# ChenyuWang-Monica/REED

Hardware: AMD Instinct MI355X
Metric: SiT-XL/2 ImageNet-256 train images/sec (higher is better)
Workload: dtype bf16

## Files before the change

include/reed_hip.h:

```cpp
#ifndef REED_HIP_H
#define REED_HIP_H
#include <stdint.h>
#ifdef __cplusplus
extern "C" {
#endif

const char* reed_last_error(void);
int reed_version(void);
int reed_half_kind(void);

int reed_gemm(int layout, int epilogue, const void* P, int64_t ldp, const void* Q, int64_t ldq,
              int M, int N, int K, void* C, int64_t ldc, void* C2, int64_t ldc2, const void* R,
              int64_t ldr, const void* bias, const void* gate, int64_t ldgate, int rows_per_gate,
              float* dbias, int accumulate, int split_k, int64_t slab_stride, void* stream);

int reed_wgrad_group(int n, const void* const* dy, const void* const* x, float* const* dw, float* const* dbias,
                     const int* n_out, const int* k_in, int tokens, int accumulate, void* stream);
int reed_wgrad_group_deal(int n, const int* n_out, const int* k_in, const int* has_bias, int cus, unsigned* items);

int reed_set_cu_reserve(int n);
int reed_planning_cus(void);
int reed_set_concurrent_comm(int on);

int reed_gemm_force_tile(int tile);
// ... 22 lines not shown

int reed_gate_bwd(const float* dx, const void* y, const void* gate, int64_t ldgate, void* dy,
                  float* part, float* part_dy, int M, int D, int T, void* stream);
int reed_transpose_bf16(const void* src, void* dst, int R, int C, void* stream);
int reed_rowsum_f32(const float* part, int R, float* ws, float* out, int N, int accumulate, void* stream);

int reed_reduce_mod_parts(const float* const* parts, const int64_t* strides, const int64_t* offs,
                          int nparts, void* dmod, int64_t lddmod, int B, int D, int chunks,
                          void* stream);

int reed_attention_fwd(const void* qkv, void* o, float* lse, int B, int T, int H, int hd,
                       void* stream);
int reed_attention_bwd(const void* qkv, const void* o, const void* d_o, const float* lse,
                       void* dqkv, int B, int T, int H, int hd, void* stream);
int64_t reed_attention_bwd_ws_floats(int B, int T, int H);
int reed_attention_bwd_ws(const void* qkv, const void* o, const void* d_o, const float* lse, void* dqkv, float* ws,
                          int B, int T, int H, int hd, void* stream);
int reed_attention_bwd_dp(const void* qkv, const void* d_o, const float* lse, const float* dpart, void* dqkv, float* ws,
                          int B, int T, int H, int hd, void* stream);

int reed_qk_norm_fwd(const void* qkv, const float* qw, const float* qb, const float* kw, const float* kb,
                     void* out, float* stats, int M, int H, int hd, float eps, void* stream);
int64_t reed_qk_norm_bwd_part_floats(int M, int H, int hd);
int reed_qk_norm_bwd(const void* dn, const void* qkv, const float* stats, const float* qw, const float* kw,
                     void* dpre, float* part, int M, int H, int hd, void* stream);

int reed_patch_embed_fwd(const float* x, const void* w, const void* bias, const float* pos,
                         float* tokens, int B, int C, int HW, int P, int D, void* stream);
int reed_patchify_bf16(const float* x, void* out, int B, int C, int HW, int P, int order, void* stream);
int64_t reed_smallk_wgrad_ws_floats(int Dw, int KS);
int reed_smallk_wgrad(const void* wide, int wide_is_f32, const void* small, float* ws, float* out,
                      float* colsum_wide, float* colsum_small, int M, int Dw, int KS, int layout,
                      int accumulate, void* stream);
int reed_timestep_sinusoid(const float* t, void* out, int B, int dim, float max_period, void* stream);
int reed_label_cond(const int64_t* labels, const uint8_t* drop, int num_classes, int table_rows, const float* table,
                    const void* t_emb, int64_t* labels_out, float* c, void* silu_c, int* err_flag, int B, int D,
                    void* stream);
int reed_label_cond_bwd(const float* dsilu_c, const float* c, const int64_t* labels_eff, void* dt_emb,
                        float* dtable, int B, int D, void* stream);
int reed_final_layer_fwd(const float* x, const void* shift, const void* scale, int64_t ldmod,
                         const void* w, const void* bias, float* out, float* mean, float* rstd,
                         int B, int T, int D, int C, int P, float eps, void* stream);
int reed_final_layer_bwd_rows(const float* dout, const float* x, const float* mean, const float* rstd,
                              const void* shift, const void* scale, int64_t ldmod, const void* w,
                              void* hbuf, void* dlin, void* dh, int B, int T, int D, int C, int P,
                              void* stream);
int reed_token_mean_fwd(const float* x, void* out, int B, int T, int D, void* stream);
int reed_token_mean_bwd(const void* dmean, float* dx, int B, int T, int D, void* stream);

int reed_sample_posterior(const float* moments, const float* eps, float* out, int B, int64_t half,
                          float scale, float bias, void* stream);
int reed_interpolant(const float* x, const float* noise, const float* t, float* xt, float* target,
                     int B, int64_t per, int path_type, void* stream);
int reed_mse_fwd(const float* out, const float* target, float* loss, int B, int64_t per, void* stream);
int reed_mse_bwd(const float* out, const float* target, const float* gscale, float* dout, int B,
                 int64_t per, void* stream);
int reed_cosine_fwd(const void* zt, const float* z, float* rowdot, float* loss, int B, int T, int Z,
                    void* stream);
int reed_cosine_bwd(const void* zt, const float* z, const float* gscale, void* dzt, int B, int T,
                    int Z, void* stream);

int reed_grad_sqnorm(const float* g, int64_t n, float* partial, int nblocks, void* stream);
int reed_clip_finalize(const float* partial, int nblocks, float max_norm, float* norm_clip, void* stream);
int reed_clip_finalize_scaled(const float* partial, int nblocks, float max_norm, float* norm_clip, float* scaler_state,
                              float growth_factor, float backoff_factor, float growth_interval, void* stream);
int reed_adamw_ema(float* p, const float* g, float* m, float* v, float* ema, void* shadow,
                   int64_t n_train, int64_t n_total, const float* norm_clip, const float* scaler_state, float lr,
                   float beta1, float beta2, float eps, float weight_decay, float bc1, float bc2, float ema_decay,
                   void* stream);
int reed_cast_bf16(const float* src, void* dst, int64_t n, void* stream);

int reed_sampler_update(const double* x_cur, const float* model_out, const double* d_prev,
                        double* d_store, double* x_next, int64_t n_elems, int cfg, double cfg_scale,
                        double dt, double w0, double w1, void* stream);
int reed_sde_update(const double* x_cur, const float* model_out, const double* eps, double* x_next,
// ... 51 lines not shown
```

reed_amd/csrc/embed.hip:

```cpp
#include "../../include/reed_hip.h"
#include "common.hpp"

namespace {

constexpr int MAXV = 5;
constexpr int NSL = 256;

__device__ __forceinline__ f32x4 ld_bf4(const bf16* p) {
  bf16x4 v = *(const bf16x4*)p;
  return f32x4{bf2f(v[0]), bf2f(v[1]), bf2f(v[2]), bf2f(v[3])};
}

__device__ __forceinline__ long patch_src(int b, int t, int k, int C, int HW, int P, int order) {
  const int G = HW / P, ph = t / G, pw = t - ph * G;
  int c, pi, pj;
  if (order == 0) { c = k / (P * P); int r = k - c * P * P; pi = r / P; pj = r - pi * P; }
  else { c = k % C; int r = k / C; pi = r / P; pj = r - pi * P; }
  return (((long)b * C + c) * HW + ph * P + pi) * HW + pw * P + pj;
}
__global__ __launch_bounds__(256) void patchify_kernel(const float* __restrict__ x, bf16* __restrict__ out, int B,
                                                       int C, int HW, int P, int order) {
  const int G = HW / P, T = G * G, K = C * P * P;
  long i = (long)blockIdx.x * 256 + threadIdx.x;
  if (i >= (long)B * T * K) return;
  int k = (int)(i % K);
  long bt = i / K;
  out[i] = f2bf(x[patch_src((int)(bt / T), (int)(bt % T), k, C, HW, P, order)]);
}

__global__ __launch_bounds__(256) void patch_embed_fwd_kernel(const float* __restrict__ x, const bf16* __restrict__ w,
                                                              const bf16* __restrict__ bias,
                                                              const float* __restrict__ pos, float* __restrict__ tok,
                                                              int B, int C, int HW, int P, int D) {
  extern __shared__ float xs[];
// ... 116 lines not shown
#pragma unroll
    for (int r = 0; r < RG; ++r) {
      ws0 += w0[r]; ws1 += w1[r];
#pragma unroll
      for (int c = 0; c < KSP / 8; ++c)
#pragma unroll
        for (int j = 0; j < 8; ++j) {
          const float f = bf2f(sv[r][c][j]);
          acc0[8 * c + j] = fmaf(w0[r], f, acc0[8 * c + j]);
          acc1[8 * c + j] = fmaf(w1[r], f, acc1[8 * c + j]);
        }
    }
  }
  if (dok) {
#pragma unroll
    for (int k = 0; k < KSP; ++k)
      if (k0 + k < KS) {
        const int kk = k0 + k;
        if (layout == 0) { wout[(long)d * KS + kk] = acc0[k]; wout[(long)(d + 1) * KS + kk] = acc1[k]; }
        else { wout[(long)kk * Dw + d] = acc0[k]; wout[(long)kk * Dw + d + 1] = acc1[k]; }
      }
    if (blockIdx.z == 0) {
      wout[(long)KS * Dw + d] = ws0;
      wout[(long)KS * Dw + d + 1] = ws1;
    }
  }
  if (blockIdx.x == 0 && blockIdx.z == 0) {
    for (int k = lane; k < KS; k += 64) {
      float ssum = 0.f;
      for (int m = mbeg; m < mend; ++m) ssum += bf2f(small[(long)m * KS + k]);
      wout[(long)KS * Dw + Dw + k] = ssum;
    }
  }
}
__global__ __launch_bounds__(256) void smallk_reduce_kernel(const float* __restrict__ ws, long stride,
                                                            float* __restrict__ o0, long n0, float* __restrict__ o1,
                                                            long n1, float* __restrict__ o2, long n2, int accumulate) {
  long i = (long)blockIdx.x * 256 + threadIdx.x;
  if (i >= n0 + n1 + n2) return;
  float* dst;
  if (i < n0) dst = o0 ? o0 + i : nullptr;
  else if (i < n0 + n1) dst = o1 ? o1 + (i - n0) : nullptr;
  else dst = o2 ? o2 + (i - n0 - n1) : nullptr;
  if (!dst) return;
  float s = accumulate ? *dst : 0.f;
  for (int z = 0; z < NSL; ++z) s += ws[(long)z * stride + i];
  *dst = s;
}

__global__ void sinusoid_kernel(const float* __restrict__ t, bf16* __restrict__ out, int B, int dim, float max_period) {
  const int half = dim / 2;
  int i = blockIdx.x * 256 + threadIdx.x;
  if (i >= B * half) return;
  int b = i / half, k = i - b * half;
  float a = (float)(-log((double)max_period)) * (float)k;
  float f = expf(a / (float)half);
  float arg = t[b] * f;
  out[(long)b * dim + k] = f2bf(cosf(arg));
  out[(long)b * dim + half + k] = f2bf(sinf(arg));
  if ((dim & 1) && k == 0) out[(long)b * dim + dim - 1] = f2bf(0.f);
}

__global__ void label_cond_kernel(const int64_t* __restrict__ labels, const uint8_t* __restrict__ drop, int num_classes,
                                  int table_rows, const float* __restrict__ table, const bf16* __restrict__ t_emb,
                                  int64_t* __restrict__ labels_out, float* __restrict__ c, bf16* __restrict__ silu_c,
                                  int* __restrict__ err, int D) {
  const int b = blockIdx.y, d = blockIdx.x * 256 + threadIdx.x;
  int64_t lab = labels[b];
  if (drop && drop[b]) lab = num_classes;
  if (lab < 0 || lab >= table_rows) {
    if (d == 0 && err) *err = 1;
    lab = 0;
  }
  if (d == 0 && labels_out) labels_out[b] = lab;
  if (d >= D) return;
  float v = bf2f(t_emb[(long)b * D + d]) + table[lab * D + d];
  c[(long)b * D + d] = v;
  silu_c[(long)b * D + d] = f2bf(silu_f(v));
}
__global__ void label_cond_bwd_kernel(const float* __restrict__ dsilu, const float* __restrict__ c,
                                      const int64_t* __restrict__ labels_eff, bf16* __restrict__ dt_emb,
                                      float* __restrict__ dtable, int B, int D) {
  const int d = blockIdx.x * 256 + threadIdx.x;
  if (d >= D) return;
  for (int b = 0; b < B; ++b) {
    float g = bfround(dsilu[(long)b * D + d]) * silu_grad_f(c[(long)b * D + d]);
    dt_emb[(long)b * D + d] = f2bf(g);
    dtable[labels_eff[b] * D + d] += g;
  }
}

__global__ __launch_bounds__(256) void final_fwd_kernel(const float* __restrict__ x, const bf16* __restrict__ shift,
                                                        const bf16* __restrict__ scale, long ldmod,
                                                        const bf16* __restrict__ w, const bf16* __restrict__ bias,
                                                        float* __restrict__ out, float* __restrict__ mean,
                                                        float* __restrict__ rstd, int B, int T, int D, int C, int P,
                                                        float eps) {
  const int row = blockIdx.x * 4 + (threadIdx.x >> 6);
  const int M = B * T;
  if (row >= M) return;
  const int lane = threadIdx.x & 63, nv = D >> 2;
  const float* xr = x + (long)row * D;
  f32x4 v[MAXV];
  float s = 0.f;
#pragma unroll
  for (int k = 0; k < MAXV; ++k) {
    int idx = lane + 64 * k;
    if (idx < nv) { v[k] = *(const f32x4*)(xr + idx * 4); s += v[k][0] + v[k][1] + v[k][2] + v[k][3]; }
  }
  const float mu = wave_sum(s) / D;
  float q = 0.f;
#pragma unroll
  for (int k = 0; k < MAXV; ++k) {
    int idx = lane + 64 * k;
    if (idx < nv) {
#pragma unroll
      for (int j = 0; j < 4; ++j) { float d = v[k][j] - mu; q += d * d; }
    }
  }
  const float r = rsqrtf(wave_sum(q) / D + eps);
  if (lane == 0 && mean) { mean[row] = mu; rstd[row] = r; }
// ... 77 lines not shown
      if (lane == 0 && mean && (u == 0 || two)) { mean[row] = mu[u]; rstd[row] = r[u]; }
      bb_[u] = row / T;
      tt_[u] = row - bb_[u] * T;
      const bf16* sc = scale + (long)bb_[u] * ldmod;
      const bf16* sh = shift + (long)bb_[u] * ldmod;
#pragma unroll
      for (int k = 0; k < MAXV; ++k) {
        int idx = lane + 64 * k;
        if (idx < nv) {
          f32x4 a = ld_bf4(sc + idx * 4), bb = ld_bf4(sh + idx * 4);
#pragma unroll
          for (int j = 0; j < 4; ++j) v[u][k][j] = bfround((v[u][k][j] - mu[u]) * r[u] * bfround(1.f + a[j]) + bb[j]);
        }
      }
    }
    for (int j = 0; j < NO; ++j) {
      float acc[2] = {0.f, 0.f};
#pragma unroll
      for (int k = 0; k < MAXV; ++k) {
        int idx = lane + 64 * k;
        if (idx < nv) {
          f32x4 wv = ld_bf4(wl + j * D + idx * 4);
#pragma unroll
          for (int u = 0; u < 2; ++u) acc[u] += v[u][k][0] * wv[0] + v[u][k][1] * wv[1] + v[u][k][2] * wv[2] + v[u][k][3] * wv[3];
        }
      }
#pragma unroll
      for (int u = 0; u < 2; ++u) acc[u] = wave_sum(acc[u]);
      if (lane == 0) {
        const float bj = bias ? bf2f(bias[j]) : 0.f;
        out[patch_src(bb_[0], tt_[0], j, C, HW, P, 1)] = bfround(acc[0] + bj);
        if (two) out[patch_src(bb_[1], tt_[1], j, C, HW, P, 1)] = bfround(acc[1] + bj);
      }
    }
  }
}

__global__ __launch_bounds__(256) void final_bwd_rows_kernel(const float* __restrict__ dout, const float* __restrict__ x,
                                                             const float* __restrict__ mean,
                                                             const float* __restrict__ rstd,
                                                             const bf16* __restrict__ shift,
                                                             const bf16* __restrict__ scale, long ldmod,
                                                             const bf16* __restrict__ w, bf16* __restrict__ hbuf,
                                                             bf16* __restrict__ dlin, bf16* __restrict__ dh, int B,
                                                             int T, int D, int C, int P) {
  extern __shared__ float dl[];
  const int wave = threadIdx.x >> 6, lane = threadIdx.x & 63, nv = D >> 2;
  const int row = blockIdx.x * 4 + wave;
  const int M = B * T, NO = P * P * C, HW = (int)(sqrtf((float)T) + 0.5f) * P;
  const bool ok = row < M;
  const int b = ok ? row / T : 0, t = ok ? row - b * T : 0;
  float* my = dl + wave * NO;
  if (ok) {
    for (int j = lane; j < NO; j += 64) {
      float g = bfround(dout[patch_src(b, t, j, C, HW, P, 1)]);
      my[j] = g;
      dlin[(long)row * NO + j] = f2bf(g);
    }
  }
  __syncthreads();
  if (!ok) return;
  const float mu = mean[row], r = rstd[row];
  const bf16* sc = scale + (long)b * ldmod;
  const bf16* sh = shift + (long)b * ldmod;
#pragma unroll
  for (int k = 0; k < MAXV; ++k) {
// ... 43 lines not shown
    }
    __builtin_amdgcn_wave_barrier();
    const float mu = mean[row], r = rstd[row];
    const bf16* sc = scale + (long)b * ldmod;
    const bf16* sh = shift + (long)b * ldmod;
#pragma unroll
    for (int k = 0; k < MAXV; ++k) {
      int idx = lane + 64 * k;
      if (idx < nv) {
        f32x4 xv = *(const f32x4*)(x + (long)row * D + idx * 4);
        f32x4 a = ld_bf4(sc + idx * 4), bb = ld_bf4(sh + idx * 4);
        bf16x4 hv, gv;
        f32x4 acc = {0, 0, 0, 0};
        for (int j = 0; j < NO; ++j) {
          f32x4 wv = ld_bf4(wl + j * D + idx * 4);
          float g = my[j];
          acc[0] += g * wv[0]; acc[1] += g * wv[1]; acc[2] += g * wv[2]; acc[3] += g * wv[3];
        }
#pragma unroll
        for (int j = 0; j < 4; ++j) {
          hv[j] = f2bf((xv[j] - mu) * r * bfround(1.f + a[j]) + bb[j]);
          gv[j] = f2bf(acc[j]);
        }
        *(bf16x4*)(hbuf + (long)row * D + idx * 4) = hv;
        *(bf16x4*)(dh + (long)row * D + idx * 4) = gv;
      }
    }
    __builtin_amdgcn_wave_barrier();
  }
}

}

extern "C" int reed_patchify_bf16(const float* x, void* out, int B, int C, int HW, int P, int order, void* stream) {
  REED_CHECK_ARG(HW % P == 0, "patchify: HW=%d not divisible by P=%d", HW, P);
  long n = (long)B * C * HW * HW;
  REED_KLAUNCH(patchify_kernel, dim3(cdiv(n, 256)), dim3(256), 0, (hipStream_t)stream, x, (bf16*)out, B, C, HW, P, order);
  REED_LAUNCH_CHECK();
  return REED_OK;
}

extern "C" int reed_patch_embed_fwd(const float* x, const void* w, const void* bias, const float* pos,
                                    float* tokens, int B, int C, int HW, int P, int D, void* stream) {
  REED_CHECK_ARG(x && w && pos && tokens, "patch_embed_fwd: null pointer");
  REED_CHECK_ARG(HW % P == 0 && (C * P * P) % 8 == 0, "patch_embed: HW=%d P=%d C=%d unsupported", HW, P, C);
  const int T = (HW / P) * (HW / P), K = C * P * P;
  if (K == PK && D % 4 == 0 && D <= 4 * PNT && ((uintptr_t)w % 16) == 0 && ((uintptr_t)pos % 16) == 0 &&
      ((uintptr_t)tokens % 16) == 0) {
    REED_KLAUNCH(patch_embed_fwd16_kernel, dim3(cdiv((long)B * T, PT)), dim3(PNT), 0, (hipStream_t)stream, x, (const bf16*)w,
                 (const bf16*)bias, pos, tokens, B, C, HW, P, D);
    REED_LAUNCH_CHECK();
    return REED_OK;
  }
  REED_KLAUNCH(patch_embed_fwd_kernel, dim3(cdiv((long)B * T, 8)), dim3(256), 8 * K * sizeof(float),
                     (hipStream_t)stream, x, (const bf16*)w, (const bf16*)bias, pos, tokens, B, C, HW, P, D);
  REED_LAUNCH_CHECK();
  return REED_OK;
}

extern "C" int64_t reed_smallk_wgrad_ws_floats(int Dw, int KS) { return (int64_t)NSL * ((int64_t)KS * Dw + Dw + KS); }

extern "C" int reed_smallk_wgrad(const void* wide, int wide_is_f32, const void* small, float* ws, float* out,
                                 float* colsum_wide, float* colsum_small, int M, int Dw, int KS, int layout,
                                 int accumulate, void* stream) {
  REED_CHECK_ARG(wide && small && ws, "smallk_wgrad: null pointer");
  REED_CHECK_ARG(KS >= 8 && KS <= 512 && KS % 8 == 0, "smallk_wgrad: KS=%d must be a multiple of 8 in 8..512", KS);
  REED_CHECK_ARG(Dw > 0 && Dw % 2 == 0, "smallk_wgrad: Dw=%d must be even", Dw);
  if (KS <= 16) {
    dim3 grid(cdiv(Dw, 128), NSL, 1);
    if (wide_is_f32) REED_KLAUNCH((smallk_wgrad_kernel<true, 16>), grid, dim3(64), 0, (hipStream_t)stream, wide, (const bf16*)small, ws, M, Dw, KS, layout);
    else REED_KLAUNCH((smallk_wgrad_kernel<false, 16>), grid, dim3(64), 0, (hipStream_t)stream, wide, (const bf16*)small, ws, M, Dw, KS, layout);
  } else {
    dim3 grid(cdiv(Dw, 128), NSL, cdiv(KS, 32));
    if (wide_is_f32) REED_KLAUNCH((smallk_wgrad_kernel<true, 32>), grid, dim3(64), 0, (hipStream_t)stream, wide, (const bf16*)small, ws, M, Dw, KS, layout);
    else REED_KLAUNCH((smallk_wgrad_kernel<false, 32>), grid, dim3(64), 0, (hipStream_t)stream, wide, (const bf16*)small, ws, M, Dw, KS, layout);
  }
  REED_LAUNCH_CHECK();
  long n0 = (long)KS * Dw, n1 = Dw, n2 = KS;
  REED_KLAUNCH(smallk_reduce_kernel, dim3(cdiv(n0 + n1 + n2, 256)), dim3(256), 0, (hipStream_t)stream, ws,
                     n0 + n1 + n2, out, n0, colsum_wide, n1, colsum_small, n2, accumulate);
  REED_LAUNCH_CHECK();
  return REED_OK;
}

extern "C" int reed_timestep_sinusoid(const float* t, void* out, int B, int dim, float max_period, void* stream) {
  REED_CHECK_ARG(t && out && dim >= 2, "timestep_sinusoid: bad args");
  REED_KLAUNCH(sinusoid_kernel, dim3(cdiv((long)B * (dim / 2), 256)), dim3(256), 0, (hipStream_t)stream, t,
                     (bf16*)out, B, dim, max_period);
  REED_LAUNCH_CHECK();
  return REED_OK;
}

extern "C" int reed_label_cond(const int64_t* labels, const uint8_t* drop, int num_classes, int table_rows,
                               const float* table, const void* t_emb, int64_t* labels_out, float* c, void* silu_c,
                               int* err_flag, int B, int D, void* stream) {
  REED_CHECK_ARG(labels && table && t_emb && c && silu_c, "label_cond: null pointer");
  REED_CHECK_ARG(table_rows >= 1 && (!drop || num_classes < table_rows),
                 "label_cond: label dropout needs a null-class row (num_classes < table_rows)");
  REED_KLAUNCH(label_cond_kernel, dim3(cdiv(D, 256), B), dim3(256), 0, (hipStream_t)stream, labels, drop,
                     num_classes, table_rows, table, (const bf16*)t_emb, labels_out, c, (bf16*)silu_c, err_flag, D);
  REED_LAUNCH_CHECK();
  return REED_OK;
}

extern "C" int reed_label_cond_bwd(const float* dsilu_c, const float* c, const int64_t* labels_eff, void* dt_emb,
                                   float* dtable, int B, int D, void* stream) {
  REED_CHECK_ARG(dsilu_c && c && labels_eff && dt_emb && dtable, "label_cond_bwd: null pointer");
  REED_KLAUNCH(label_cond_bwd_kernel, dim3(cdiv(D, 256)), dim3(256), 0, (hipStream_t)stream, dsilu_c, c,
                     labels_eff, (bf16*)dt_emb, dtable, B, D);
  REED_LAUNCH_CHECK();
  return REED_OK;
}

extern "C" int reed_final_layer_fwd(const float* x, const void* shift, const void* scale, int64_t ldmod,
                                    const void* w, const void* bias, float* out, float* mean, float* rstd,
                                    int B, int T, int D, int C, int P, float eps, void* stream) {
  REED_CHECK_ARG(x && shift && scale && w && out, "final_layer_fwd: null pointer");
  REED_CHECK_ARG(D % 4 == 0 && D <= 256 * MAXV, "final_layer: D=%d unsupported", D);
  int G = (int)(sqrtf((float)T) + 0.5f);
  REED_CHECK_ARG(G * G == T, "final_layer: T=%d is not a square grid", T);
  const long wbytes = (long)P * P * C * D * sizeof(bf16);
  if (wbytes <= 64 * 1024 && (P * P * C * D) % 8 == 0 && ((uintptr_t)w % 16) == 0) {
    REED_KLAUNCH(final_fwd_lds_kernel, dim3(cdiv((long)B * T, FR)), dim3(256), (size_t)wbytes, (hipStream_t)stream, x,
                 (const bf16*)shift, (const bf16*)scale, (long)ldmod, (const bf16*)w, (const bf16*)bias, out, mean, rstd, B, T, D, C, P,
                 eps);
    REED_LAUNCH_CHECK();
    return REED_OK;
  }
  REED_KLAUNCH(final_fwd_kernel, dim3(cdiv((long)B * T, 4)), dim3(256), 0, (hipStream_t)stream, x,
                     (const bf16*)shift, (const bf16*)scale, (long)ldmod, (const bf16*)w, (const bf16*)bias, out, mean,
                     rstd, B, T, D, C, P, eps);
  REED_LAUNCH_CHECK();
  return REED_OK;
}

extern "C" int reed_final_layer_bwd_rows(const float* dout, const float* x, const float* mean, const float* rstd,
                                         const void* shift, const void* scale, int64_t ldmod, const void* w,
                                         void* hbuf, void* dlin, void* dh, int B, int T, int D, int C, int P,
                                         void* stream) {
  REED_CHECK_ARG(dout && x && mean && rstd && shift && scale && w && hbuf && dlin && dh, "final_layer_bwd_rows: null pointer");
  REED_CHECK_ARG(D % 4 == 0 && D <= 256 * MAXV, "final_layer: D=%d unsupported", D);
  REED_CHECK_ARG(B > 0 && T > 0, "final_layer_bwd_rows: bad B=%d T=%d", B, T);
  int G = (int)(sqrtf((float)T) + 0.5f);
  REED_CHECK_ARG(G * G == T, "final_layer_bwd_rows: T=%d is not a square grid", T);
  const int NO = P * P * C;
  const long wb = (long)NO * D * sizeof(bf16);
  if (wb + 4 * NO * (long)sizeof(float) <= 64 * 1024 && (NO * D) % 8 == 0 && ((uintptr_t)w % 16) == 0) {
    REED_KLAUNCH(final_bwd_rows_lds_kernel, dim3(cdiv((long)B * T, FR)), dim3(256), (size_t)(wb + 4 * NO * sizeof(float)),
                 (hipStream_t)stream, dout, x, mean, rstd, (const bf16*)shift, (const bf16*)scale, (long)ldmod, (const bf16*)w,
                 (bf16*)hbuf, (bf16*)dlin, (bf16*)dh, B, T, D, C, P);
    REED_LAUNCH_CHECK();
    return REED_OK;
  }
  REED_KLAUNCH(final_bwd_rows_kernel, dim3(cdiv((long)B * T, 4)), dim3(256), 4 * NO * sizeof(float),
                     (hipStream_t)stream, dout, x, mean, rstd, (const bf16*)shift, (const bf16*)scale, (long)ldmod,
                     (const bf16*)w, (bf16*)hbuf, (bf16*)dlin, (bf16*)dh, B, T, D, C, P);
  REED_LAUNCH_CHECK();
  return REED_OK;
}
```

reed_amd/ops.py:

```python
import contextlib
import ctypes

import math

import torch

from . import _lib

NT, NN, TN = 0, 1, 2
TN_TALL, TN_WIDE = 3, 4
(EPI_BF16, EPI_GELU, EPI_SILU, EPI_GATE_RES, EPI_DGELU, EPI_DSILU, EPI_F32, EPI_ADDF32_RB, EPI_ATOMIC_F32, EPI_QGELU,
 EPI_RES_BF16, EPI_GELU_ERF, EPI_LS_RES, EPI_BF16_DOT, EPI_GELU_G, EPI_SILU_G, EPI_MUL, EPI_SWIGLU) = range(18)
SWIGLU_GROUP = 8


def _p(t):
    if t is None:
        return None
    if isinstance(t, int):
        return t
    return t.data_ptr()


def _stream():
# ... 436 lines not shown
        return False
    _lib.check(rc, "reed_gemm", L)
    return True


def attention_bwd_ws_floats(B, T, H):
    return int(_lib.load(_PRECISION).reed_attention_bwd_ws_floats(B, T, H))


def qk_norm_fwd(qkv, qw, qb, kw, kb, out, stats, M, H, hd, eps=1e-5):
    _call("reed_qk_norm_fwd", _p(qkv), _p(qw), _p(qb), _p(kw), _p(kb), _p(out), _p(stats), M, H, hd, eps, _stream())


def qk_norm_part_floats(M, H, hd):
    return int(_lib.load().reed_qk_norm_bwd_part_floats(M, H, hd))


def qk_norm_bwd(dn, qkv, stats, qw, kw, dpre, part, M, H, hd):
    _call("reed_qk_norm_bwd", _p(dn), _p(qkv), _p(stats), _p(qw), _p(kw), _p(dpre), _p(part), M, H, hd, _stream())


def patch_embed_fwd(x, w, bias, pos, tokens, B, C, HW, P, D):
    _call("reed_patch_embed_fwd", _p(x), _p(w), _p(bias), _p(pos), _p(tokens), B, C, HW, P, D, _stream())


def patchify_bf16(x, out, B, C, HW, P, order):
    _call("reed_patchify_bf16", _p(x), _p(out), B, C, HW, P, order, _stream())


def smallk_ws_floats(Dw, KS):
    return int(_lib.load().reed_smallk_wgrad_ws_floats(Dw, KS))


def smallk_wgrad(wide, wide_is_f32, small, ws, out, colsum_wide, colsum_small, M, Dw, KS, layout, accumulate):
    _call("reed_smallk_wgrad", _p(wide), int(wide_is_f32), _p(small), _p(ws), _p(out), _p(colsum_wide),
          _p(colsum_small), M, Dw, KS, layout, int(accumulate), _stream())


def timestep_sinusoid(t, out, B, dim=256, max_period=10000.0):
    _call("reed_timestep_sinusoid", _p(t), _p(out), B, dim, max_period, _stream())


def label_cond(labels, drop, num_classes, table, t_emb, labels_out, c, silu_c, B, D, table_rows=None, err=None):
    if table_rows is None:
        table_rows = num_classes + 1
    _call("reed_label_cond", _p(labels), _p(drop), num_classes, table_rows, _p(table), _p(t_emb), _p(labels_out), _p(c),
          _p(silu_c), _p(err), B, D, _stream())


def label_cond_bwd(dsilu_c, c, labels_eff, dt_emb, dtable, B, D):
    _call("reed_label_cond_bwd", _p(dsilu_c), _p(c), _p(labels_eff), _p(dt_emb), _p(dtable), B, D, _stream())


def final_layer_fwd(x, shift, scale, ldmod, w, bias, out, mean, rstd, B, T, D, C, P, eps=1e-6):
    _call("reed_final_layer_fwd", _p(x), _p(shift), _p(scale), ldmod, _p(w), _p(bias), _p(out), _p(mean), _p(rstd),
          B, T, D, C, P, eps, _stream())


def final_layer_bwd_rows(dout, x, mean, rstd, shift, scale, ldmod, w, hbuf, dlin, dh, B, T, D, C, P):
    _call("reed_final_layer_bwd_rows", _p(dout), _p(x), _p(mean), _p(rstd), _p(shift), _p(scale), ldmod, _p(w),
          _p(hbuf), _p(dlin), _p(dh), B, T, D, C, P, _stream())


def clip_im2col(img, out, B, S, P, Kp):
    _call("reed_clip_im2col", _p(img), _p(out), B, S, P, Kp, _stream())


def clip_tokens(patches, cls, pos, out, B, T, D):
    _call("reed_clip_tokens", _p(patches), _p(cls), _p(pos), _p(out), B, T, D, _stream())


def ln_affine_bf16(x, w, b, out, M, D, eps=1e-5):
    _call("reed_ln_affine_bf16", _p(x), _p(w), _p(b), _p(out), M, D, eps, _stream())


def sample_posterior(moments, eps, out, B, half, scale, bias):
    _call("reed_sample_posterior", _p(moments), _p(eps), _p(out), B, half, float(scale), float(bias), _stream())


def interpolant(x, noise, t, xt, target, B, per, path_type):
    _call("reed_interpolant", _p(x), _p(noise), _p(t), _p(xt), _p(target), B, per, path_type, _stream())


def mse_fwd(out, target, loss, B, per):
    _call("reed_mse_fwd", _p(out), _p(target), _p(loss), B, per, _stream())


# ... 104 lines not shown
```

Before: 1338.

## Add faster kernels for small-K wgrad, label-cond backward, and final-layer forward

Adds three new kernels that become the default path: a small-K weight-gradient kernel with a double-buffered LDS stage and a register ring of wide rows, a label-conditioning backward that chains same-label samples so each table row is written by one thread instead of serial scatter, and a final-layer forward that holds the fp32 weight in up to 144 KiB of LDS, runs a persistent grid and reduces outputs across lanes with a shuffle butterfly. Form arguments keep the old kernels selectable. These are small ops in the SiT step, so the effect on the whole step is bounded, and the larger LDS use and bigger unrolled register footprint may lower occupancy.

```diff
diff --git a/include/reed_hip.h b/include/reed_hip.h
--- a/include/reed_hip.h
+++ b/include/reed_hip.h
@@ -78,15 +78,23 @@
 int reed_smallk_wgrad(const void* wide, int wide_is_f32, const void* small, float* ws, float* out,
                       float* colsum_wide, float* colsum_small, int M, int Dw, int KS, int layout,
                       int accumulate, void* stream);
+int reed_smallk_wgrad_form(const void* wide, int wide_is_f32, const void* small, float* ws, float* out,
+                           float* colsum_wide, float* colsum_small, int M, int Dw, int KS, int layout,
+                           int accumulate, int form, void* stream);
 int reed_timestep_sinusoid(const float* t, void* out, int B, int dim, float max_period, void* stream);
 int reed_label_cond(const int64_t* labels, const uint8_t* drop, int num_classes, int table_rows, const float* table,
                     const void* t_emb, int64_t* labels_out, float* c, void* silu_c, int* err_flag, int B, int D,
                     void* stream);
 int reed_label_cond_bwd(const float* dsilu_c, const float* c, const int64_t* labels_eff, void* dt_emb,
                         float* dtable, int B, int D, void* stream);
+int reed_label_cond_bwd_form(const float* dsilu_c, const float* c, const int64_t* labels_eff, void* dt_emb,
+                             float* dtable, int B, int D, int form, void* stream);
 int reed_final_layer_fwd(const float* x, const void* shift, const void* scale, int64_t ldmod,
                          const void* w, const void* bias, float* out, float* mean, float* rstd,
                          int B, int T, int D, int C, int P, float eps, void* stream);
+int reed_final_layer_fwd_form(const float* x, const void* shift, const void* scale, int64_t ldmod,
+                              const void* w, const void* bias, float* out, float* mean, float* rstd,
+                              int B, int T, int D, int C, int P, float eps, int form, void* stream);
 int reed_final_layer_bwd_rows(const float* dout, const float* x, const float* mean, const float* rstd,
                               const void* shift, const void* scale, int64_t ldmod, const void* w,
                               void* hbuf, void* dlin, void* dh, int B, int T, int D, int C, int P,
diff --git a/reed_amd/csrc/embed.hip b/reed_amd/csrc/embed.hip
--- a/reed_amd/csrc/embed.hip
+++ b/reed_amd/csrc/embed.hip
@@ -1,5 +1,6 @@
 #include "../../include/reed_hip.h"
 #include "common.hpp"
+#include <type_traits>
 
 namespace {
 
@@ -182,6 +183,156 @@
       wout[(long)KS * Dw + Dw + k] = ssum;
     }
   }
+}
+constexpr int SKW = 8;
+template <bool WIDE_F32, int KSP>
+__global__ __launch_bounds__(SKW * 64) void smallk_wgrad_wide_kernel(const void* __restrict__ wide, const bf16* __restrict__ small,
+                                                                     float* __restrict__ ws, int M, int Dw, int KS, int layout) {
+  constexpr bool W4 = WIDE_F32 || sizeof(bf16) == 4;
+  constexpr int CPL = KSP == 16 ? 4 : 2;
+  constexpr int RPR = W4 ? CPL : CPL / 2;
+  constexpr int RG = 4, CH = KSP == 16 ? 64 / RPR : 16, NG = CH / RG, SV = CH * KSP > 512 ? CH * KSP / 512 : 1;
+  typedef __attribute__((ext_vector_type(CPL))) float FV;
+  typedef __attribute__((ext_vector_type(CPL))) bf16 HV;
+  typedef typename std::conditional<WIDE_F32, FV, HV>::type WV;
+  __shared__ __attribute__((aligned(16))) float sm[2][CH * KSP];
+  const int wave = threadIdx.x >> 6, lane = threadIdx.x & 63, nthr = blockDim.x;
+  const int d = (blockIdx.x * (nthr >> 6) + wave) * (64 * CPL) + CPL * lane;
+  const int slice = blockIdx.y;
+  const int per = (M + NSL - 1) / NSL;
+  const int mbeg = slice * per, mend = min(M, mbeg + per);
+  float* wout = ws + (long)slice * ((long)KS * Dw + Dw + KS);
+  const bool dok = d < Dw;
+  const bool wact = d - CPL * lane < Dw;
+  const int dc = dok ? d : 0;
+  const int kc = KS >> 3;
+  f32x2 acc[KSP][CPL / 2];
+#pragma unroll
+  for (int k = 0; k < KSP; ++k)
+#pragma unroll
+    for (int p = 0; p < CPL / 2; ++p) acc[k][p] = f32x2{0.f, 0.f};
+  float cw[CPL];
+#pragma unroll
+  for (int e = 0; e < CPL; ++e) cw[e] = 0.f;
+  float cs = 0.f;
+  const bool cs_wave = blockIdx.x == 0 && wave == 0;
+
+  auto ldw = [&](int m) -> WV {
+    const long off = (long)min(m, mend - 1) * Dw + dc;
+    if constexpr (WIDE_F32) return *(const WV*)((const float*)wide + off);
+    else return *(const WV*)((const bf16*)wide + off);
+  };
+  auto stage_load = [&](int m0, bf16x8 (&st)[SV]) {
+#pragma unroll
+    for (int i = 0; i < SV; ++i) {
+      const int v = threadIdx.x + i * nthr;
+      if (v < CH * kc) st[i] = *(const bf16x8*)(small + (long)min(m0 + v / kc, mend - 1) * KS + 8 * (v % kc));
+    }
+  };
+  auto stage_store = [&](float* sb, const bf16x8 (&st)[SV]) {
+#pragma unroll
+    for (int i = 0; i < SV; ++i) {
+      const int v = threadIdx.x + i * nthr;
+      if (v < CH * kc) {
+        float* p = sb + (v / kc) * KSP + 8 * (v % kc);
+        *(f32x4*)p = f32x4{bf2f(st[i][0]), bf2f(st[i][1]), bf2f(st[i][2]), bf2f(st[i][3])};
+        *(f32x4*)(p + 4) = f32x4{bf2f(st[i][4]), bf2f(st[i][5]), bf2f(st[i][6]), bf2f(st[i][7])};
+      }
+    }
+  };
+
+  if (mbeg < mend) {
+    WV ring[NG][RG];
+    bf16x8 st[SV];
+    stage_load(mbeg, st);
+    stage_store(sm[0], st);
+    if (wact) {
+#pragma unroll
+      for (int g = 0; g < NG; ++g)
+#pragma unroll
+        for (int r = 0; r < RG; ++r) ring[g][r] = ldw(mbeg + g * RG + r);
+    }
+    __syncthreads();
+    for (int m0 = mbeg, buf = 0; m0 < mend; m0 += CH, buf ^= 1) {
+      const bool more = m0 + CH < mend;
+      if (more) stage_load(m0 + CH, st);
+      const float* sb = sm[buf];
+      if (wact) {
+        constexpr int UPR = KSP / 16, NU = CH * UPR;
+        f32x4 fu[2][4];
+        auto ldu = [&](int u, f32x4 (&f)[4]) {
+          const float* p = sb + (u / UPR) * KSP + (u % UPR) * 16;
+#pragma unroll
+          for (int q = 0; q < 4; ++q) f[q] = *(const f32x4*)(p + 4 * q);
+        };
+        ldu(0, fu[0]);
+#pragma unroll
+        for (int g = 0; g < NG; ++g) {
+          if (m0 + g * RG < mend) {
+#pragma unroll
+            for (int r = 0; r < RG; ++r) {
+              const WV raw = ring[g][r];
+              float w[CPL];
+#pragma unroll
+              for (int e = 0; e < CPL; ++e) {
+                if constexpr (WIDE_F32) w[e] = bfround(raw[e]);
+                else w[e] = bf2f(raw[e]);
+                if (m0 + g * RG + r >= mend) w[e] = 0.f;
+                cw[e] += w[e];
+              }
+#pragma unroll
+              for (int hh = 0; hh < UPR; ++hh) {
+                const int u = (g * RG + r) * UPR + hh;
+                if (u + 1 < NU) ldu(u + 1, fu[(u + 1) & 1]);
+#pragma unroll
+                for (int q = 0; q < 4; ++q)
+#pragma unroll
+                  for (int j = 0; j < 4; ++j) {
+                    const float fv = fu[u & 1][q][j];
+                    const f32x2 ff = {fv, fv};
+#pragma unroll
+                    for (int p = 0; p < CPL / 2; ++p)
+                      acc[16 * hh + 4 * q + j][p] = __builtin_elementwise_fma(f32x2{w[2 * p], w[2 * p + 1]}, ff, acc[16 * hh + 4 * q + j][p]);
+                  }
+                __builtin_amdgcn_sched_barrier(0);
+              }
+            }
+            if (more) {
+#pragma unroll
+              for (int r = 0; r < RG; ++r) ring[g][r] = ldw(m0 + CH + g * RG + r);
+            }
+          }
+        }
+      }
+      if (cs_wave && lane < KS) {
+        const int n = min(CH, mend - m0);
+        for (int r = 0; r < n; ++r) cs += sb[r * KSP + lane];
+      }
+      if (more) stage_store(sm[buf ^ 1], st);
+      __syncthreads();
+    }
+  }
+  if (dok) {
+    if (layout == 0) {
+#pragma unroll
+      for (int e = 0; e < CPL; ++e)
+#pragma unroll
+        for (int q = 0; q < KSP / 4; ++q)
+          if (4 * q < KS)
+            *(f32x4*)(wout + (long)(d + e) * KS + 4 * q) = f32x4{acc[4 * q][e >> 1][e & 1], acc[4 * q + 1][e >> 1][e & 1],
+                                                                 acc[4 * q + 2][e >> 1][e & 1], acc[4 * q + 3][e >> 1][e & 1]};
+    } else {
+#pragma unroll
+      for (int k = 0; k < KSP; ++k)
+        if (k < KS) {
+#pragma unroll
+          for (int p = 0; p < CPL / 2; ++p) *(f32x2*)(wout + (long)k * Dw + d + 2 * p) = acc[k][p];
+        }
+    }
+#pragma unroll
+    for (int p = 0; p < CPL / 2; ++p) *(f32x2*)(wout + (long)KS * Dw + d + 2 * p) = f32x2{cw[2 * p], cw[2 * p + 1]};
+  }
+  if (cs_wave && lane < KS) wout[(long)KS * Dw + Dw + lane] = cs;
 }
 __global__ __launch_bounds__(256) void smallk_reduce_kernel(const float* __restrict__ ws, long stride,
                                                             float* __restrict__ o0, long n0, float* __restrict__ o1,
@@ -237,6 +388,46 @@
     float g = bfround(dsilu[(long)b * D + d]) * silu_grad_f(c[(long)b * D + d]);
     dt_emb[(long)b * D + d] = f2bf(g);
     dtable[labels_eff[b] * D + d] += g;
+  }
+}
+constexpr int LC = 8, LNT = 1024;
+__global__ __launch_bounds__(LNT) void label_cond_bwd_chain_kernel(const float* __restrict__ dsilu, const float* __restrict__ c,
+                                                                   const int64_t* __restrict__ labels_eff, bf16* __restrict__ dt_emb,
+                                                                   float* __restrict__ dtable, int B, int D) {
+  extern __shared__ __attribute__((aligned(16))) char lc_raw[];
+  float* fa = (float*)lc_raw;
+  float* fb = fa + (long)B * LC;
+  int* lab = (int*)(fb + (long)B * LC);
+  int* nxt = lab + B;
+  int* head = nxt + B;
+  const int d0 = blockIdx.x * LC;
+  for (int b = threadIdx.x; b < B; b += LNT) { lab[b] = (int)labels_eff[b]; head[b] = 1; }
+  for (int i = threadIdx.x; i < B * LC; i += LNT) {
+    const int b = i / LC, e = i - b * LC, d = d0 + e;
+    if (d < D) {
+      const float a = bfround(dsilu[(long)b * D + d]), s = silu_grad_f(c[(long)b * D + d]);
+      fa[i] = a;
+      fb[i] = s;
+      dt_emb[(long)b * D + d] = f2bf(a * s);
+    }
+  }
+  __syncthreads();
+  for (int b = threadIdx.x; b < B; b += LNT) {
+    const int l = lab[b];
+    int n = -1;
+    for (int j = b + 1; j < B; ++j)
+      if (lab[j] == l) { n = j; break; }
+    nxt[b] = n;
+    if (n >= 0) head[n] = 0;
+  }
+  __syncthreads();
+  for (int i = threadIdx.x; i < B * LC; i += LNT) {
+    const int b = i / LC, e = i - b * LC, d = d0 + e;
+    if (d >= D || !head[b]) continue;
+    float* dst = dtable + (long)lab[b] * D + d;
+    float s = *dst;
+    for (int j = b; j >= 0; j = nxt[j]) s = fmaf(fb[j * LC + e], fa[j * LC + e], s);
+    *dst = s;
   }
 }
 
@@ -380,6 +571,156 @@
         out[patch_src(bb_[0], tt_[0], j, C, HW, P, 1)] = bfround(acc[0] + bj);
         if (two) out[patch_src(bb_[1], tt_[1], j, C, HW, P, 1)] = bfround(acc[1] + bj);
       }
+    }
+  }
+}
+
+template <int NO>
+__global__ __launch_bounds__(256, 2) void final_fwd_regs_kernel(const float* __restrict__ x, const bf16* __restrict__ shift,
+                                                                const bf16* __restrict__ scale, long ldmod,
+                                                                const bf16* __restrict__ w, const bf16* __restrict__ bias,
+                                                                float* __restrict__ out, float* __restrict__ mean,
+                                                                float* __restrict__ rstd, int B, int T, int D, int C, int P,
+                                                                float eps, int fr) {
+#pragma clang fp contract(off)
+  extern __shared__ __attribute__((aligned(16))) char wl_raw[];
+  float* wl = (float*)wl_raw;
+  const int M = B * T;
+  for (int i = threadIdx.x * 8; i < NO * D; i += 256 * 8) {
+    const bf16x8 w8 = *(const bf16x8*)(w + i);
+    *(f32x4*)(wl + i) = f32x4{bf2f(w8[0]), bf2f(w8[1]), bf2f(w8[2]), bf2f(w8[3])};
+    *(f32x4*)(wl + i + 4) = f32x4{bf2f(w8[4]), bf2f(w8[5]), bf2f(w8[6]), bf2f(w8[7])};
+  }
+  __syncthreads();
+  const int wave = threadIdx.x >> 6, lane = threadIdx.x & 63, nv = D >> 2, kv = (nv + 63) >> 6;
+  const int HW = (int)(sqrtf((float)T) + 0.5f) * P;
+  constexpr int NV2 = 2 * NO, LG = NO == 32 ? 6 : 5;
+  const int rend = min(M, (blockIdx.x + 1) * fr);
+  f32x4 v[2][MAXV], vn[2][MAXV];
+  auto load_pair = [&](int row0, f32x4 (&dst)[2][MAXV]) {
+#pragma unroll
+    for (int u = 0; u < 2; ++u) {
+      const float* xr = x + (long)min(row0 + u, M - 1) * D;
+#pragma unroll
+      for (int k = 0; k < MAXV; ++k) {
+        const int idx = lane + 64 * k;
+        if (idx < nv) dst[u][k] = *(const f32x4*)(xr + idx * 4);
+      }
+    }
+  };
+  int row0 = blockIdx.x * fr + 2 * wave;
+  if (row0 < rend) load_pair(row0, vn);
+  for (; row0 < rend; row0 += 8) {
+    const bool two = row0 + 1 < M;
+#pragma unroll
+    for (int u = 0; u < 2; ++u)
+#pragma unroll
+      for (int k = 0; k < MAXV; ++k) v[u][k] = vn[u][k];
+    float s[2] = {0.f, 0.f};
+#pragma unroll
+    for (int u = 0; u < 2; ++u)
+#pragma unroll
+      for (int k = 0; k < MAXV; ++k) {
+        int idx = lane + 64 * k;
+        if (idx < nv) s[u] += v[u][k][0] + v[u][k][1] + v[u][k][2] + v[u][k][3];
+      }
+    float mu[2], r[2];
+#pragma unroll
+    for (int u = 0; u < 2; ++u) mu[u] = wave_sum(s[u]) / D;
+    float q[2] = {0.f, 0.f};
+#pragma unroll
+    for (int u = 0; u < 2; ++u)
+#pragma unroll
+      for (int k = 0; k < MAXV; ++k) {
+        int idx = lane + 64 * k;
+        if (idx < nv) {
+#pragma unroll
+          for (int j = 0; j < 4; ++j) { float d = v[u][k][j] - mu[u]; q[u] += d * d; }
+        }
+      }
+#pragma unroll
+    for (int u = 0; u < 2; ++u) r[u] = rsqrtf(wave_sum(q[u]) / D + eps);
+    int bb_[2], tt_[2];
+    f32x2 h[MAXV][4];
+#pragma unroll
+    for (int u = 0; u < 2; ++u) {
+      const int row = row0 + (u && two ? 1 : 0);
+      if (lane == 0 && mean && (u == 0 || two)) { mean[row] = mu[u]; rstd[row] = r[u]; }
+      bb_[u] = row / T;
+      tt_[u] = row - bb_[u] * T;
+      const bf16* sc = scale + (long)bb_[u] * ldmod;
+      const bf16* sh = shift + (long)bb_[u] * ldmod;
+#pragma unroll
+      for (int k = 0; k < MAXV; ++k) {
+        int idx = lane + 64 * k;
+        if (idx < nv) {
+          f32x4 a = ld_bf4(sc + idx * 4), bb = ld_bf4(sh + idx * 4);
+#pragma unroll
+          for (int j = 0; j < 4; ++j) {
+            float y = fmaf((v[u][k][j] - mu[u]) * r[u], bfround(1.f + a[j]), bb[j]);
+            asm volatile("" : "+v"(y));
+            h[k][j][u] = bfround(y);
+          }
+        } else {
+#pragma unroll
+          for (int j = 0; j < 4; ++j) h[k][j][u] = 0.f;
+        }
+      }
+    }
+    if (row0 + 8 < rend) load_pair(row0 + 8, vn);
+    f32x2 acc[NO];
+#pragma unroll
+    for (int j = 0; j < NO; ++j) acc[j] = f32x2{0.f, 0.f};
+#pragma unroll
+    for (int k = 0; k < MAXV; ++k) {
+      if (k < kv) {
+        const int idx = lane + 64 * k;
+        const float* wk = wl + (idx < nv ? idx : 0) * 4;
+        f32x4 wq[2][4];
+#pragma unroll
+        for (int e = 0; e < 4; ++e) wq[0][e] = *(const f32x4*)(wk + e * D);
+#pragma unroll
+        for (int jb = 0; jb < NO / 4; ++jb) {
+          if (jb + 1 < NO / 4) {
+#pragma unroll
+            for (int e = 0; e < 4; ++e) wq[(jb + 1) & 1][e] = *(const f32x4*)(wk + (4 * jb + 4 + e) * D);
+          }
+#pragma unroll
+          for (int e = 0; e < 4; ++e) {
+            const f32x4 wb = wq[jb & 1][e];
+            f32x2 t = h[k][0] * f32x2{wb[0], wb[0]};
+            t = __builtin_elementwise_fma(h[k][1], f32x2{wb[1], wb[1]}, t);
+            t = __builtin_elementwise_fma(h[k][2], f32x2{wb[2], wb[2]}, t);
+            t = __builtin_elementwise_fma(h[k][3], f32x2{wb[3], wb[3]}, t);
+            acc[4 * jb + e] = acc[4 * jb + e] + t;
+          }
+          __builtin_amdgcn_sched_barrier(0);
+        }
+      }
+    }
+    float a[NV2];
+#pragma unroll
+    for (int j = 0; j < NO; ++j) { a[j] = acc[j][0]; a[NO + j] = acc[j][1]; }
+#pragma unroll
+    for (int lvl = 0; lvl < 6; ++lvl) {
+      const int o = 32 >> lvl, n = NV2 >> lvl;
+      if (n > 1) {
+        const bool up = lane & o;
+#pragma unroll
+        for (int i = 0; i < n / 2; ++i) {
+          float lo = a[i], hi = a[i + n / 2];
+          asm volatile("" : "+v"(lo), "+v"(hi));
+          const float keep = up ? hi : lo, send = up ? lo : hi;
+          a[i] = keep + __shfl_xor(send, o, 64);
+        }
+      } else {
+        a[0] = a[0] + __shfl_xor(a[0], o, 64);
+      }
+    }
+    const int vi = lane >> (6 - LG), u = vi / NO, j = vi - u * NO;
+    if ((lane & ((1 << (6 - LG)) - 1)) == 0 && (u == 0 || two)) {
+      const float bj = bias ? bf2f(bias[j]) : 0.f;
+      out[patch_src(u ? bb_[1] : bb_[0], u ? tt_[1] : tt_[0], j, C, HW, P, 1)] = bfround(a[0] + bj);
     }
   }
 }
@@ -489,6 +830,8 @@
 
 }
 
+int reed_num_cus();
+
 extern "C" int reed_patchify_bf16(const float* x, void* out, int B, int C, int HW, int P, int order, void* stream) {
   REED_CHECK_ARG(HW % P == 0, "patchify: HW=%d not divisible by P=%d", HW, P);
   long n = (long)B * C * HW * HW;
@@ -517,13 +860,27 @@
 
 extern "C" int64_t reed_smallk_wgrad_ws_floats(int Dw, int KS) { return (int64_t)NSL * ((int64_t)KS * Dw + Dw + KS); }
 
-extern "C" int reed_smallk_wgrad(const void* wide, int wide_is_f32, const void* small, float* ws, float* out,
-                                 float* colsum_wide, float* colsum_small, int M, int Dw, int KS, int layout,
-                                 int accumulate, void* stream) {
+static int smallk_wgrad_launch(const void* wide, int wide_is_f32, const void* small, float* ws, float* out, float* colsum_wide,
+                               float* colsum_small, int M, int Dw, int KS, int layout, int accumulate, int form, void* stream) {
   REED_CHECK_ARG(wide && small && ws, "smallk_wgrad: null pointer");
   REED_CHECK_ARG(KS >= 8 && KS <= 512 && KS % 8 == 0, "smallk_wgrad: KS=%d must be a multiple of 8 in 8..512", KS);
   REED_CHECK_ARG(Dw > 0 && Dw % 2 == 0, "smallk_wgrad: Dw=%d must be even", Dw);
-  if (KS <= 16) {
+  REED_CHECK_ARG(form >= 0 && form <= 2, "smallk_wgrad: form=%d is not 0, 1 or 2", form);
+  const size_t wrow = 4 * (wide_is_f32 ? sizeof(float) : sizeof(bf16));
+  const bool wide_ok = M > 0 && KS <= 32 && Dw % 4 == 0 && ((uintptr_t)wide % wrow) == 0 && ((uintptr_t)ws % 16) == 0 &&
+                       ((uintptr_t)small % (8 * sizeof(bf16))) == 0;
+  REED_CHECK_ARG(form != 2 || wide_ok, "smallk_wgrad: the one-pass form needs KS <= 32, Dw %% 4 == 0 and aligned arrays (KS=%d Dw=%d)", KS, Dw);
+  if (form != 1 && wide_ok) {
+    const int ncg = cdiv(Dw, KS <= 16 ? 256 : 128), gx = cdiv(ncg, SKW), nw = cdiv(ncg, gx);
+    dim3 grid(gx, NSL, 1), block(nw * 64);
+    if (KS <= 16) {
+      if (wide_is_f32) REED_KLAUNCH((smallk_wgrad_wide_kernel<true, 16>), grid, block, 0, (hipStream_t)stream, wide, (const bf16*)small, ws, M, Dw, KS, layout);
+      else REED_KLAUNCH((smallk_wgrad_wide_kernel<false, 16>), grid, block, 0, (hipStream_t)stream, wide, (const bf16*)small, ws, M, Dw, KS, layout);
+    } else {
+      if (wide_is_f32) REED_KLAUNCH((smallk_wgrad_wide_kernel<true, 32>), grid, block, 0, (hipStream_t)stream, wide, (const bf16*)small, ws, M, Dw, KS, layout);
+      else REED_KLAUNCH((smallk_wgrad_wide_kernel<false, 32>), grid, block, 0, (hipStream_t)stream, wide, (const bf16*)small, ws, M, Dw, KS, layout);
+    }
+  } else if (KS <= 16) {
     dim3 grid(cdiv(Dw, 128), NSL, 1);
     if (wide_is_f32) REED_KLAUNCH((smallk_wgrad_kernel<true, 16>), grid, dim3(64), 0, (hipStream_t)stream, wide, (const bf16*)small, ws, M, Dw, KS, layout);
     else REED_KLAUNCH((smallk_wgrad_kernel<false, 16>), grid, dim3(64), 0, (hipStream_t)stream, wide, (const bf16*)small, ws, M, Dw, KS, layout);
@@ -538,6 +895,18 @@
                      n0 + n1 + n2, out, n0, colsum_wide, n1, colsum_small, n2, accumulate);
   REED_LAUNCH_CHECK();
   return REED_OK;
+}
+
+extern "C" int reed_smallk_wgrad(const void* wide, int wide_is_f32, const void* small, float* ws, float* out,
+                                 float* colsum_wide, float* colsum_small, int M, int Dw, int KS, int layout,
+                                 int accumulate, void* stream) {
+  return smallk_wgrad_launch(wide, wide_is_f32, small, ws, out, colsum_wide, colsum_small, M, Dw, KS, layout, accumulate, 0, stream);
+}
+
+extern "C" int reed_smallk_wgrad_form(const void* wide, int wide_is_f32, const void* small, float* ws, float* out,
+                                      float* colsum_wide, float* colsum_small, int M, int Dw, int KS, int layout,
+                                      int accumulate, int form, void* stream) {
+  return smallk_wgrad_launch(wide, wide_is_f32, small, ws, out, colsum_wide, colsum_small, M, Dw, KS, layout, accumulate, form, stream);
 }
 
 extern "C" int reed_timestep_sinusoid(const float* t, void* out, int B, int dim, float max_period, void* stream) {
@@ -560,24 +929,76 @@
   return REED_OK;
 }
 
+static int label_cond_bwd_launch(const float* dsilu_c, const float* c, const int64_t* labels_eff, void* dt_emb, float* dtable, int B,
+                                 int D, int form, void* stream) {
+  REED_CHECK_ARG(dsilu_c && c && labels_eff && dt_emb && dtable, "label_cond_bwd: null pointer");
+  REED_CHECK_ARG(form >= 0 && form <= 2, "label_cond_bwd: form=%d is not 0, 1 or 2", form);
+  const long lds = (long)B * (2 * LC + 3) * 4;
+  const bool chain_ok = B > 0 && D > 0 && lds <= 64 * 1024;
+  REED_CHECK_ARG(form != 2 || chain_ok, "label_cond_bwd: the chain form holds %d bytes of LDS per sample: B=%d is too large", (2 * LC + 3) * 4, B);
+  if (form != 1 && chain_ok)
+    REED_KLAUNCH(label_cond_bwd_chain_kernel, dim3(cdiv(D, LC)), dim3(LNT), (size_t)lds, (hipStream_t)stream, dsilu_c, c, labels_eff,
+                 (bf16*)dt_emb, dtable, B, D);
+  else
+    REED_KLAUNCH(label_cond_bwd_kernel, dim3(cdiv(D, 256)), dim3(256), 0, (hipStream_t)stream, dsilu_c, c,
+                       labels_eff, (bf16*)dt_emb, dtable, B, D);
+  REED_LAUNCH_CHECK();
+  return REED_OK;
+}
+
 extern "C" int reed_label_cond_bwd(const float* dsilu_c, const float* c, const int64_t* labels_eff, void* dt_emb,
                                    float* dtable, int B, int D, void* stream) {
-  REED_CHECK_ARG(dsilu_c && c && labels_eff && dt_emb && dtable, "label_cond_bwd: null pointer");
-  REED_KLAUNCH(label_cond_bwd_kernel, dim3(cdiv(D, 256)), dim3(256), 0, (hipStream_t)stream, dsilu_c, c,
-                     labels_eff, (bf16*)dt_emb, dtable, B, D);
-  REED_LAUNCH_CHECK();
-  return REED_OK;
-}
-
-extern "C" int reed_final_layer_fwd(const float* x, const void* shift, const void* scale, int64_t ldmod,
-                                    const void* w, const void* bias, float* out, float* mean, float* rstd,
-                                    int B, int T, int D, int C, int P, float eps, void* stream) {
+  return label_cond_bwd_launch(dsilu_c, c, labels_eff, dt_emb, dtable, B, D, 0, stream);
+}
+
+extern "C" int reed_label_cond_bwd_form(const float* dsilu_c, const float* c, const int64_t* labels_eff, void* dt_emb,
+                                        float* dtable, int B, int D, int form, void* stream) {
+  return label_cond_bwd_launch(dsilu_c, c, labels_eff, dt_emb, dtable, B, D, form, stream);
+}
+
+static int final_layer_fwd_launch(const float* x, const void* shift, const void* scale, int64_t ldmod, const void* w, const void* bias,
+                                  float* out, float* mean, float* rstd, int B, int T, int D, int C, int P, float eps, int form,
+                                  void* stream) {
   REED_CHECK_ARG(x && shift && scale && w && out, "final_layer_fwd: null pointer");
   REED_CHECK_ARG(D % 4 == 0 && D <= 256 * MAXV, "final_layer: D=%d unsupported", D);
+  REED_CHECK_ARG(form >= 0 && form <= 2, "final_layer_fwd: form=%d is not 0, 1 or 2", form);
   int G = (int)(sqrtf((float)T) + 0.5f);
   REED_CHECK_ARG(G * G == T, "final_layer: T=%d is not a square grid", T);
-  const long wbytes = (long)P * P * C * D * sizeof(bf16);
-  if (wbytes <= 64 * 1024 && (P * P * C * D) % 8 == 0 && ((uintptr_t)w % 16) == 0) {
+  const int NO = P * P * C;
+  const long wbytes = (long)NO * D * sizeof(bf16);
+  const bool fits = wbytes <= 64 * 1024 && (NO * D) % 8 == 0 && ((uintptr_t)w % 16) == 0;
+  const long wfbytes = (long)NO * D * sizeof(float);
+  const bool regs_ok = (NO == 16 || NO == 32) && wfbytes <= 144 * 1024 && ((uintptr_t)w % 16) == 0 && B > 0 && T > 0;
+  REED_CHECK_ARG(form != 2 || regs_ok, "final_layer_fwd: the register form needs 16 or 32 outputs and an aligned weight of at most 144 KiB as fp32 (NO=%d D=%d)", NO, D);
+#if defined(REED_FP32)
+  const bool regs = form == 2;
+#else
+  const bool regs = form != 1 && regs_ok;
+#endif
+  if (regs) {
+    static bool attr_set = false;
+    if (!attr_set) {
+      hipError_t e = hipFuncSetAttribute((const void*)final_fwd_regs_kernel<16>, hipFuncAttributeMaxDynamicSharedMemorySize, 144 * 1024);
+      if (e == hipSuccess) e = hipFuncSetAttribute((const void*)final_fwd_regs_kernel<32>, hipFuncAttributeMaxDynamicSharedMemorySize, 144 * 1024);
+      if (e != hipSuccess) { reed_set_error("final_layer_fwd: cannot reserve 144 KiB LDS: %s", hipGetErrorString(e)); return (int)e; }
+      attr_set = true;
+    }
+    const long groups = cdiv((long)B * T, 8);
+    const long resident = (long)reed_num_cus() * (wfbytes <= 80 * 1024 ? 2 : 1);
+    const int nblk = (int)(groups < resident ? groups : resident);
+    const int fr = 8 * cdiv(groups, nblk);
+    if (NO == 16)
+      REED_KLAUNCH(final_fwd_regs_kernel<16>, dim3(cdiv((long)B * T, fr)), dim3(256), (size_t)wfbytes, (hipStream_t)stream, x,
+                   (const bf16*)shift, (const bf16*)scale, (long)ldmod, (const bf16*)w, (const bf16*)bias, out, mean, rstd, B, T, D, C, P,
+                   eps, fr);
+    else
+      REED_KLAUNCH(final_fwd_regs_kernel<32>, dim3(cdiv((long)B * T, fr)), dim3(256), (size_t)wfbytes, (hipStream_t)stream, x,
+                   (const bf16*)shift, (const bf16*)scale, (long)ldmod, (const bf16*)w, (const bf16*)bias, out, mean, rstd, B, T, D, C, P,
+                   eps, fr);
+    REED_LAUNCH_CHECK();
+    return REED_OK;
+  }
+  if (fits) {
     REED_KLAUNCH(final_fwd_lds_kernel, dim3(cdiv((long)B * T, FR)), dim3(256), (size_t)wbytes, (hipStream_t)stream, x,
                  (const bf16*)shift, (const bf16*)scale, (long)ldmod, (const bf16*)w, (const bf16*)bias, out, mean, rstd, B, T, D, C, P,
                  eps);
@@ -589,6 +1010,18 @@
                      rstd, B, T, D, C, P, eps);
   REED_LAUNCH_CHECK();
   return REED_OK;
+}
+
+extern "C" int reed_final_layer_fwd(const float* x, const void* shift, const void* scale, int64_t ldmod,
+                                    const void* w, const void* bias, float* out, float* mean, float* rstd,
+                                    int B, int T, int D, int C, int P, float eps, void* stream) {
+  return final_layer_fwd_launch(x, shift, scale, ldmod, w, bias, out, mean, rstd, B, T, D, C, P, eps, 0, stream);
+}
+
+extern "C" int reed_final_layer_fwd_form(const float* x, const void* shift, const void* scale, int64_t ldmod,
+                                         const void* w, const void* bias, float* out, float* mean, float* rstd,
+                                         int B, int T, int D, int C, int P, float eps, int form, void* stream) {
+  return final_layer_fwd_launch(x, shift, scale, ldmod, w, bias, out, mean, rstd, B, T, D, C, P, eps, form, stream);
 }
 
 extern "C" int reed_final_layer_bwd_rows(const float* dout, const float* x, const float* mean, const float* rstd,
diff --git a/reed_amd/ops.py b/reed_amd/ops.py
--- a/reed_amd/ops.py
+++ b/reed_amd/ops.py
@@ -492,7 +492,11 @@
     return int(_lib.load().reed_smallk_wgrad_ws_floats(Dw, KS))
 
 
-def smallk_wgrad(wide, wide_is_f32, small, ws, out, colsum_wide, colsum_small, M, Dw, KS, layout, accumulate):
+def smallk_wgrad(wide, wide_is_f32, small, ws, out, colsum_wide, colsum_small, M, Dw, KS, layout, accumulate, form=0):
+    if form:
+        _call("reed_smallk_wgrad_form", _p(wide), int(wide_is_f32), _p(small), _p(ws), _p(out), _p(colsum_wide),
+              _p(colsum_small), M, Dw, KS, layout, int(accumulate), form, _stream())
+        return
     _call("reed_smallk_wgrad", _p(wide), int(wide_is_f32), _p(small), _p(ws), _p(out), _p(colsum_wide),
           _p(colsum_small), M, Dw, KS, layout, int(accumulate), _stream())
 
@@ -508,11 +512,18 @@
           _p(silu_c), _p(err), B, D, _stream())
 
 
-def label_cond_bwd(dsilu_c, c, labels_eff, dt_emb, dtable, B, D):
+def label_cond_bwd(dsilu_c, c, labels_eff, dt_emb, dtable, B, D, form=0):
+    if form:
+        _call("reed_label_cond_bwd_form", _p(dsilu_c), _p(c), _p(labels_eff), _p(dt_emb), _p(dtable), B, D, form, _stream())
+        return
     _call("reed_label_cond_bwd", _p(dsilu_c), _p(c), _p(labels_eff), _p(dt_emb), _p(dtable), B, D, _stream())
 
 
-def final_layer_fwd(x, shift, scale, ldmod, w, bias, out, mean, rstd, B, T, D, C, P, eps=1e-6):
+def final_layer_fwd(x, shift, scale, ldmod, w, bias, out, mean, rstd, B, T, D, C, P, eps=1e-6, form=0):
+    if form:
+        _call("reed_final_layer_fwd_form", _p(x), _p(shift), _p(scale), ldmod, _p(w), _p(bias), _p(out), _p(mean), _p(rstd),
+              B, T, D, C, P, eps, form, _stream())
+        return
     _call("reed_final_layer_fwd", _p(x), _p(shift), _p(scale), ldmod, _p(w), _p(bias), _p(out), _p(mean), _p(rstd),
           B, T, D, C, P, eps, _stream())
 
```

Measured after the change: 1342, median of 6. Within noise of the previous version (+0.3%).
